# shubhamchandak94/Spring

Measured on AMD Instinct MI355X. Metric: Mreads/s through reorder stage, higher is better.
Workload: dtype u64; 1 GPU; 100000000 x 150 bp single-end synthetic reads per GPU (uniform genome 600000000 bp, 25x coverage, 1.0% substitutions, 50% reverse-complemented), inputs resident in HBM as .dna records; reads_per_gpu=100000000, read_len=150, chains=65536, num_thr=8, parallelism=single GPU, unmatched=13958636, singletons=12720853, rounds=1984, chain_groups=2

## Files before the change

### include/spring_reorder.h

```cpp
#ifndef SPRING_REORDER_H_
#define SPRING_REORDER_H_

#include <stddef.h>
#include <stdint.h>

#ifdef __cplusplus
extern "C" {
#endif

#define SPRING_REORDER_E_ARG (-1)
#define SPRING_REORDER_E_IO (-2)
#define SPRING_REORDER_E_HIP (-3)
#define SPRING_REORDER_E_STATE (-4)

typedef struct spring_reorder_ctx spring_reorder_ctx;

typedef struct {
  int32_t device;
  uint32_t num_chains;
  int32_t num_thr;
  int32_t collect_stats;
  int32_t time_search;
  int32_t force_literal_update;
  int32_t rounds_per_sync;
// ... 92 lines not shown
int spring_reorder_mg_slice(spring_reorder_ctx *ctx, void **d_prop, size_t *slice_off, size_t *slice_bytes,
                            size_t *total_bytes);
int spring_reorder_mg_slices(spring_reorder_ctx *ctx, void **d_prop, size_t slice_off[2], size_t slice_bytes[2],
                             size_t *total_bytes, uint32_t *count);
int spring_reorder_mg_apply(spring_reorder_ctx *ctx, int32_t check_alive, uint32_t *alive);
int spring_reorder_mg_end(spring_reorder_ctx *ctx);
int spring_reorder_debug_check_seed_state(spring_reorder_ctx *ctx, int32_t group, uint64_t *violations);
int spring_reorder_mg_exchange_virtual(spring_reorder_ctx **ctxs, uint32_t world);

#define SPRING_RCCL_ID_BYTES 128
typedef struct spring_mg_comm spring_mg_comm;
typedef int (*spring_mg_allgather_fn)(void *host_buf, size_t slice_off, size_t slice_bytes, size_t total_bytes,
                                      void *user);
int spring_mg_rccl_unique_id(void *id128);
int spring_mg_comm_create_rccl(spring_mg_comm **comm, int32_t device, const void *id128, uint32_t rank, uint32_t world);
int spring_mg_comm_create_host(spring_mg_comm **comm, spring_mg_allgather_fn fn, void *user, uint32_t rank,
                               uint32_t world);
void spring_mg_comm_destroy(spring_mg_comm *comm);
int spring_reorder_mg_run(spring_reorder_ctx *ctx, spring_mg_comm *comm, uint32_t total_chains);

int spring_reorder_finalize(spring_reorder_ctx *ctx);

int spring_reorder_get_stats(spring_reorder_ctx *ctx, spring_reorder_stats *st);

int spring_reorder_download(spring_reorder_ctx *ctx, uint32_t *order, char *rc, char *flag, int64_t *pos,
                            uint16_t *rlen, uint32_t *order_s, uint64_t *tid_off, uint64_t *tid_off_s);
int spring_reorder_tid_split(spring_reorder_ctx *ctx, uint64_t *mid, uint64_t *mid_s);

int spring_reorder_emit_dna(spring_reorder_ctx *ctx, int32_t tid, uint8_t *dst, size_t cap, size_t *nbytes);

int spring_reorder_dict_lookup(spring_reorder_ctx *ctx, int32_t which, const uint64_t *keys, uint32_t nkeys,
                               uint32_t *bin_size, uint32_t *bin_ids, size_t ids_cap);

int spring_reorder_download_reads(spring_reorder_ctx *ctx, uint64_t *limbs , uint16_t *len);

int spring_order_invert_se(const uint32_t *order, uint32_t n, uint32_t *order_array, double *kernel_ms);
int spring_order_invert_pe(const uint32_t *order, uint32_t n, uint32_t *order_array, double *kernel_ms);
int spring_order_correct(uint32_t *order, uint64_t m, const uint32_t *order_N, uint32_t nN, uint32_t n_clean,
                         double *kernel_ms);
int spring_order_pe_encode(const uint32_t *order, uint32_t n, uint32_t *new_order, double *kernel_ms);

int spring_fastq_reorder(const uint8_t *fastq, size_t nbytes, const uint32_t *order, uint32_t n, uint8_t *out,
                         size_t out_cap, size_t *out_bytes, double *kernel_ms);

#define SPRING_SYNTH_REPEATS 0x80000000u
#define SPRING_SYNTH_PAIRED 0x40000000u
#define SPRING_SYNTH_GENOMIC 0x20000000u
size_t spring_synth_dna_bytes(uint32_t n, uint32_t L);
int spring_synth_dna_host(uint8_t *dst, uint32_t n, uint32_t L, uint64_t G, uint64_t seed, uint32_t err_ppm);
int spring_synth_genome_host(uint8_t *dst, uint64_t G, uint64_t seed, uint32_t flags);
int spring_synth_dna_device(void *d_dst, uint32_t n, uint32_t L, uint64_t G, uint64_t seed, uint32_t err_ppm);
int spring_reorder_load_synth(spring_reorder_ctx *ctx, uint32_t n, uint32_t L, uint64_t G, uint64_t seed,
                              uint32_t err_ppm);
int spring_reorder_download_dna(spring_reorder_ctx *ctx, uint8_t *dst, size_t cap);

#ifdef __cplusplus
}
#endif
#endif
```

### spring_amd/_lib.py

```python
import ctypes as C
import os

HERE = os.path.dirname(os.path.abspath(__file__))
LIB_PATH = os.environ.get("SPRING_AMD_LIB") or os.path.join(HERE, "lib", "libspring_reorder_hip.so")

EXPORTS = [
    "spring_reorder_default_opts", "spring_reorder_last_error", "spring_reorder_trim_pool", "spring_reorder_run", "spring_reorder_create",
    "spring_reorder_destroy", "spring_reorder_load_dna", "spring_reorder_load_dna_device",
    "spring_reorder_build_dict", "spring_reorder_run_chains", "spring_reorder_auto_chains", "spring_reorder_finalize",
    "spring_reorder_mg_begin", "spring_reorder_mg_search", "spring_reorder_mg_slice", "spring_reorder_mg_slices",
    "spring_reorder_mg_apply",
    "spring_reorder_mg_end", "spring_reorder_mg_exchange_virtual", "spring_reorder_debug_check_seed_state",
    "spring_mg_rccl_unique_id", "spring_mg_comm_create_rccl", "spring_mg_comm_create_host", "spring_mg_comm_destroy",
    "spring_reorder_mg_run",
    "spring_reorder_get_stats", "spring_reorder_download", "spring_reorder_tid_split", "spring_reorder_emit_dna",
    "spring_reorder_dict_lookup", "spring_reorder_download_reads", "spring_synth_dna_bytes",
    "spring_reorder_load_fastq", "spring_reorder_fastq_N",
    "spring_order_invert_se", "spring_order_invert_pe", "spring_order_correct", "spring_order_pe_encode",
    "spring_fastq_reorder",
    "spring_synth_dna_host", "spring_synth_genome_host", "spring_synth_dna_device", "spring_reorder_load_synth", "spring_reorder_download_dna",
    "spring_encoder_create", "spring_encoder_destroy", "spring_encoder_set_split_tables", "spring_encoder_encode_reorder", "spring_encoder_download",
    "spring_encoder_download_seq_packed", "spring_encoder_get_info", "spring_reorder_encode_run", "spring_encoder_encode_host", "spring_encoder_run",
]

STREAMS_EXPORTS = [
    "spring_streams_create", "spring_streams_destroy", "spring_streams_from_encoder", "spring_streams_from_host",
    "spring_streams_download", "spring_streams_get_info", "spring_streams_run",
]
STREAMS_NUM = 9

DECODE_EXPORTS = [
    "spring_decode_create", "spring_decode_destroy", "spring_decode_seq_from_encoder", "spring_decode_seq_from_host",
    "spring_decode_seq_from_files", "spring_decode_from_streams", "spring_decode_from_host", "spring_decode_from_files",
    "spring_decode_download", "spring_decode_get_info",
]

QUALID_EXPORTS = [
    "spring_qualid_create", "spring_qualid_destroy", "spring_qualid_order_from_host", "spring_qualid_order_from_encoder",
    "spring_qualid_from_fastq", "spring_qualid_from_lines", "spring_qualid_download", "spring_qualid_get_info",
    "spring_quality_table", "spring_id_pattern",
]

FASTQ_OUT_EXPORTS = [
    "spring_fastq_out_create", "spring_fastq_out_destroy", "spring_fastq_out_assemble", "spring_fastq_out_download",
    "spring_fastq_out_write", "spring_fastq_out_get_info",
]

GZIP_EXPORTS = [
    "spring_gzip_create", "spring_gzip_destroy", "spring_gzip_set_chunk_bytes", "spring_gzip_from_fastq_out",
# ... 189 lines not shown
    L.spring_reorder_last_error.restype = C.c_char_p
    L.spring_reorder_trim_pool.restype = None
    L.spring_reorder_run.argtypes = [C.c_char_p, C.c_uint32, C.c_int32, C.c_int32, C.c_uint32, C.c_uint32,
                                     C.POINTER(Opts)]
    L.spring_reorder_create.argtypes = [C.POINTER(vp), C.POINTER(Opts)]
    L.spring_reorder_destroy.argtypes = [vp]
    L.spring_reorder_destroy.restype = None
    L.spring_reorder_load_dna.argtypes = [vp, u8p, C.c_size_t, C.c_uint32, C.c_uint32]
    L.spring_reorder_load_dna_device.argtypes = [vp, vp, C.c_size_t, C.c_uint32, C.c_uint32, C.c_int32]
    L.spring_reorder_build_dict.argtypes = [vp]
    L.spring_reorder_run_chains.argtypes = [vp]
    L.spring_reorder_auto_chains.argtypes = [vp, C.POINTER(C.c_uint32), C.POINTER(C.c_int32)]
    L.spring_reorder_finalize.argtypes = [vp]
    L.spring_reorder_mg_begin.argtypes = [vp, C.c_uint32, C.c_uint32, C.c_uint32, vp]
    L.spring_reorder_mg_search.argtypes = [vp]
    L.spring_reorder_mg_slice.argtypes = [vp, C.POINTER(vp), C.POINTER(C.c_size_t), C.POINTER(C.c_size_t), C.POINTER(C.c_size_t)]
    L.spring_reorder_mg_slices.argtypes = [vp, C.POINTER(vp), C.POINTER(C.c_size_t), C.POINTER(C.c_size_t), C.POINTER(C.c_size_t),
                                           C.POINTER(C.c_uint32)]
    L.spring_reorder_debug_check_seed_state.argtypes = [vp, C.c_int32, C.POINTER(C.c_uint64)]
    L.spring_reorder_mg_apply.argtypes = [vp, C.c_int32, C.POINTER(C.c_uint32)]
    L.spring_reorder_mg_end.argtypes = [vp]
    L.spring_reorder_mg_exchange_virtual.argtypes = [C.POINTER(vp), C.c_uint32]
    L.spring_mg_rccl_unique_id.argtypes = [vp]
    L.spring_mg_comm_create_rccl.argtypes = [C.POINTER(vp), C.c_int32, vp, C.c_uint32, C.c_uint32]
    L.spring_mg_comm_create_host.argtypes = [C.POINTER(vp), MG_ALLGATHER_FN, vp, C.c_uint32, C.c_uint32]
    L.spring_mg_comm_destroy.argtypes = [vp]
    L.spring_mg_comm_destroy.restype = None
    L.spring_reorder_mg_run.argtypes = [vp, vp, C.c_uint32]
    L.spring_reorder_get_stats.argtypes = [vp, C.POINTER(Stats)]
    L.spring_reorder_download.argtypes = [vp] + [vp] * 8
    L.spring_reorder_tid_split.argtypes = [vp, vp, vp]
    L.spring_reorder_emit_dna.argtypes = [vp, C.c_int32, u8p, C.c_size_t, C.POINTER(C.c_size_t)]
    L.spring_reorder_dict_lookup.argtypes = [vp, C.c_int32, vp, C.c_uint32, vp, vp, C.c_size_t]
    L.spring_reorder_download_reads.argtypes = [vp, vp, vp]
    L.spring_reorder_load_fastq.argtypes = [vp, vp, C.c_size_t, vp, C.c_size_t, C.POINTER(FastqInfo)]
    L.spring_reorder_fastq_N.argtypes = [vp, C.c_int32, vp, C.c_size_t, C.POINTER(C.c_size_t), vp, C.POINTER(C.c_uint32)]
    L.spring_order_invert_se.argtypes = [vp, C.c_uint32, vp, C.POINTER(C.c_double)]
    L.spring_order_invert_pe.argtypes = [vp, C.c_uint32, vp, C.POINTER(C.c_double)]
    L.spring_fastq_reorder.argtypes = [u8p, C.c_size_t, vp, C.c_uint32, u8p, C.c_size_t, C.POINTER(C.c_size_t),
                                       C.POINTER(C.c_double)]
    L.spring_order_pe_encode.argtypes = [vp, C.c_uint32, vp, C.POINTER(C.c_double)]
    L.spring_order_correct.argtypes = [vp, C.c_uint64, vp, C.c_uint32, C.c_uint32, C.POINTER(C.c_double)]
    L.spring_synth_dna_bytes.restype = C.c_size_t
    L.spring_synth_dna_bytes.argtypes = [C.c_uint32, C.c_uint32]
    L.spring_synth_dna_host.argtypes = [u8p, C.c_uint32, C.c_uint32, C.c_uint64, C.c_uint64, C.c_uint32]
    L.spring_synth_genome_host.argtypes = [u8p, C.c_uint64, C.c_uint64, C.c_uint32]
    L.spring_synth_dna_device.argtypes = [vp, C.c_uint32, C.c_uint32, C.c_uint64, C.c_uint64, C.c_uint32]
    L.spring_reorder_load_synth.argtypes = [vp, C.c_uint32, C.c_uint32, C.c_uint64, C.c_uint64, C.c_uint32]
    L.spring_reorder_download_dna.argtypes = [vp, u8p, C.c_size_t]
    L.spring_encoder_create.argtypes = [C.c_int32, C.POINTER(vp)]
    L.spring_encoder_destroy.argtypes = [vp]
    L.spring_encoder_destroy.restype = None
    L.spring_encoder_encode_reorder.argtypes = [vp, vp, u8p, C.c_uint64, vp, C.c_uint32, C.POINTER(EncoderInfo)]
    L.spring_encoder_download.argtypes = [vp] + [vp] * 9
    L.spring_encoder_download_seq_packed.argtypes = [vp, vp, vp]
    L.spring_encoder_encode_host.argtypes = [vp, C.c_uint32, C.c_int32, vp, u8p, C.c_uint64, vp, vp, vp, vp, vp, u8p,
                                             C.c_uint64, vp, C.c_uint32, u8p, C.c_uint64, vp, C.c_uint32,
                                             C.POINTER(EncoderInfo)]
    L.spring_encoder_run.argtypes = [C.c_char_p, C.c_uint32, C.c_int32, C.c_uint32, C.c_uint32, C.c_int32,
                                     C.POINTER(EncoderInfo)]
    L.spring_encoder_get_info.argtypes = [vp, C.POINTER(EncoderInfo)]
    L.spring_reorder_encode_run.argtypes = [C.c_char_p, C.c_uint32, C.c_int32, C.c_int32, C.c_uint32, C.c_uint32,
                                            C.c_uint32, C.POINTER(Opts), C.POINTER(EncoderInfo)]
    L.spring_streams_create.argtypes = [C.c_int32, C.POINTER(vp)]
    L.spring_streams_destroy.argtypes = [vp]
    L.spring_streams_destroy.restype = None
# ... 104 lines not shown
```

### spring_amd/csrc/dict_build.h

```cpp
#ifndef SPRING_DICT_BUILD_H_
#define SPRING_DICT_BUILD_H_

#include "reorder_device.h"

namespace sr {

bool launch_unpack_keys(hipStream_t st, const uint8_t *dna, uint32_t n, int L, int W, int S, uint32_t rec_fixed,
                        uint64_t *reads, uint16_t *lens, uint32_t *bad_len, int dstart0, int dend0, int dstart1, int dend1,
                        uint64_t *keys0, uint32_t *vals0, uint64_t *keys1, uint32_t *vals1);

constexpr int TAB_WRITE_LG = 10;
inline int tab_write_lg(int bshift) { return 64 - bshift < TAB_WRITE_LG ? 64 - bshift : TAB_WRITE_LG; }
inline uint32_t tab_write_blocks(int bshift) { return (uint32_t)(1ull << (64 - bshift - tab_write_lg(bshift))); }
void launch_tab_partition(hipStream_t st, const uint64_t *h0, uint32_t nk0, const uint64_t *h1, uint32_t nk1, int bshift,
                          uint32_t *part);
constexpr uint32_t TAB_OVF_SLOTS = 8;
void launch_tab_write(hipStream_t st, const uint64_t *h0, uint32_t nk0, const uint64_t *h1, uint32_t nk1,
                      const uint32_t *part, DictBuild d0, DictBuild d1, uint4 *fpt, int bshift, uint32_t *ovf,
                      uint32_t *ovf_blk, uint32_t *ovf_cnt);
void launch_tab_overflow_blocks(hipStream_t st, const uint64_t *h0, uint32_t nk0, const uint64_t *h1, DictBuild d0,
                                DictBuild d1, uint32_t *fpt, int bshift, const uint32_t *ovf_blk, const uint32_t *ovf_cnt);
void launch_tab_overflow_pairs(hipStream_t st, const uint64_t *h0, uint32_t nk0, const uint64_t *h1, DictBuild d0,
                               DictBuild d1, uint32_t *fpt, int bshift, const uint32_t *ovf, uint32_t novf);

constexpr uint32_t PRES_DROP_CTRS = 1024;
void launch_pres_insert(hipStream_t st, const uint64_t *h0, uint32_t nk0, const uint64_t *h1, uint32_t nk1, int wl, uint32_t *pres,
                        int lgb, uint32_t *drops);

}

#endif
```

### spring_amd/csrc/dict_build.hip

```cpp
#include <hip/hip_runtime.h>

#include "dict_build.h"
#include "strand_filter.h"

namespace sr {

__device__ __forceinline__ uint64_t db_mix64(uint64_t x) {
  x ^= x >> 33; x *= 0xff51afd7ed558ccdull; x ^= x >> 33; x *= 0xc4ceb9fe1a85ec53ull; x ^= x >> 33;
  return x;
}
__device__ __forceinline__ uint64_t db_unmix64(uint64_t x) {
  x ^= x >> 33; x *= 0x9cb4b2f8129337dbull; x ^= x >> 33; x *= 0x4f74430c22a54005ull; x ^= x >> 33;
  return x;
}
__device__ __forceinline__ uint32_t db_fp30_of(uint64_t h) {
  const uint32_t f = (uint32_t)h & 0x3fffffffu;
  return f == 0u ? 1u : f == 0x3fffffffu ? 0x3ffffffeu : f;
}

__global__ __launch_bounds__(256) void k_unpack_fixed_keys(const uint8_t *__restrict__ dna, uint32_t n, int L, int W, int lgS,
                                                           uint32_t rec, uint64_t *__restrict__ reads,
                                                           uint16_t *__restrict__ lens, uint32_t *__restrict__ bad_len,
                                                           int dstart0, int klen0, int dstart1, int klen1,
                                                           uint64_t *__restrict__ keys0, uint32_t *__restrict__ vals0,
// ... 233 lines not shown
  if (t >= ovf[0]) return;
  tab_overflow_insert(ovf[1u + t], h0, nk0, h1, d0, d1, fpt, bshift);
}

void launch_tab_partition(hipStream_t st, const uint64_t *h0, uint32_t nk0, const uint64_t *h1, uint32_t nk1, int bshift,
                          uint32_t *part) {
  const uint32_t nblk = tab_write_blocks(bshift);
  const uint64_t nt = 2ull * ((uint64_t)nblk + 1);
  hipLaunchKernelGGL(k_tab_partition, dim3((unsigned)((nt + 255) / 256)), dim3(256), 0, st, h0, nk0, h1, nk1, bshift,
                     tab_write_lg(bshift), nblk, part);
}
void launch_tab_write(hipStream_t st, const uint64_t *h0, uint32_t nk0, const uint64_t *h1, uint32_t nk1,
                      const uint32_t *part, DictBuild d0, DictBuild d1, uint4 *fpt, int bshift, uint32_t *ovf,
                      uint32_t *ovf_blk, uint32_t *ovf_cnt) {
  const uint32_t nblk = tab_write_blocks(bshift);
  hipLaunchKernelGGL(k_tab_write, dim3(nblk), dim3(TAB_WRITE_THREADS), 0, st, h0, nk0, h1, nk1, part, nblk, d0, d1, fpt, bshift,
                     tab_write_lg(bshift), ovf, ovf_blk, ovf_cnt);
}
void launch_tab_overflow_blocks(hipStream_t st, const uint64_t *h0, uint32_t nk0, const uint64_t *h1, DictBuild d0,
                                DictBuild d1, uint32_t *fpt, int bshift, const uint32_t *ovf_blk, const uint32_t *ovf_cnt) {
  const uint32_t nblk = tab_write_blocks(bshift);
  const uint64_t nt = (uint64_t)nblk * TAB_OVF_SLOTS;
  hipLaunchKernelGGL(k_tab_overflow_blocks, dim3((unsigned)((nt + 255) / 256)), dim3(256), 0, st, h0, nk0, h1, d0, d1, fpt, bshift,
                     nblk, ovf_blk, ovf_cnt);
}
void launch_tab_overflow_pairs(hipStream_t st, const uint64_t *h0, uint32_t nk0, const uint64_t *h1, DictBuild d0,
                               DictBuild d1, uint32_t *fpt, int bshift, const uint32_t *ovf, uint32_t novf) {
  if (!novf) return;
  hipLaunchKernelGGL(k_tab_overflow_pairs, dim3((novf + 255) / 256), dim3(256), 0, st, h0, nk0, h1, d0, d1, fpt, bshift, ovf);
}

__global__ __launch_bounds__(256) void k_pres_insert(const uint64_t *__restrict__ h0, uint32_t nk0, const uint64_t *__restrict__ h1,
                                                     uint32_t nk1, int wl, uint32_t *__restrict__ pres, int lgb,
                                                     uint32_t *__restrict__ drops) {
  __shared__ uint32_t s_drop;
  if (threadIdx.x == 0) s_drop = 0u;
  __syncthreads();
  const uint64_t t = (uint64_t)blockIdx.x * blockDim.x + threadIdx.x;
  if (t < (uint64_t)nk0 + nk1) {
    const int l = t >= nk0 ? 1 : 0;
    const uint64_t key = db_unmix64(l ? h1[t - nk0] : h0[t]);
    uint32_t flags;
    const uint64_t hc = sf::mix64(sf::canon_and_flags(key, wl, l, flags));
    const uint32_t fp = sf::fp_of(hc), word = (fp << 4) | flags;
    uint32_t *bk = pres + 4ull * sf::bucket_of(hc, lgb);
    bool placed = false;
    for (int sl = 0; sl < 4 && !placed; sl++) {
      uint32_t old = __hip_atomic_load(bk + sl, __ATOMIC_RELAXED, __HIP_MEMORY_SCOPE_AGENT);
      if (old == 0u) old = atomicCAS(bk + sl, 0u, word);
      if (old == 0u) placed = true;
      else if ((old >> 4) == fp) {
        if ((old & word & 15u) != (word & 15u)) atomicOr(bk + sl, word & 15u);
        placed = true;
      }
    }
    if (!placed) atomicAdd(&s_drop, 1u);
  }
  __syncthreads();
  if (threadIdx.x == 0 && s_drop) atomicAdd(drops + (blockIdx.x & (PRES_DROP_CTRS - 1u)), s_drop);
}
void launch_pres_insert(hipStream_t st, const uint64_t *h0, uint32_t nk0, const uint64_t *h1, uint32_t nk1, int wl, uint32_t *pres,
                        int lgb, uint32_t *drops) {
  const uint64_t nt = (uint64_t)nk0 + nk1;
  if (!nt) return;
  hipLaunchKernelGGL(k_pres_insert, dim3((unsigned)((nt + 255) / 256)), dim3(256), 0, st, h0, nk0, h1, nk1, wl, pres, lgb, drops);
}

}
```

### spring_amd/csrc/reorder_pipeline.cpp

```cpp
#include <hip/hip_runtime.h>
#include <dlfcn.h>

#include <algorithm>
#include <system_error>
#include <thread>
#include <memory>
#include <atomic>
#include <chrono>
#include <cstdarg>
#include <cstdio>
#include <cstdlib>
#include <cstring>
#include <map>
#include <mutex>
#include <new>
#include <stdexcept>
#include <string>
#include <unordered_map>
#include <vector>
#include <zlib.h>

#include "reorder_device.h"
#include "dict_build.h"
#include "reorder_internal.h"
// ... 965 lines not shown
  HIPCHK(hipStreamSynchronize(ctx->st));
  if (!ctx->n) return 0;
  if (limbs)
    HIPCHK(hipMemcpy2D(limbs, (size_t)ctx->W * 8, ctx->d_reads, (size_t)ctx->S * 8, (size_t)ctx->W * 8, ctx->n,
                       hipMemcpyDeviceToHost));
  if (len) HIPCHK(hipMemcpy(len, ctx->d_lens, (size_t)ctx->n * 2, hipMemcpyDeviceToHost));
  return 0;
}

static uint64_t pow2ceil(uint64_t x) {
  uint64_t p = 1;
  while (p < x) p <<= 1;
  return p;
}

static double now_ms() {
  return std::chrono::duration<double, std::milli>(std::chrono::steady_clock::now().time_since_epoch()).count();
}
#define DBG_T(label)                                                                         \
  do {                                                                                       \
    if (dbg) { (void)hipStreamSynchronize(st); double t_ = now_ms(); fprintf(stderr, "[dict] %-14s %8.2f ms\n", label, t_ - t_last); t_last = t_; } \
  } while (0)

static TabView tab_view(const spring_reorder_ctx *ctx) {
  TabView t;
  t.buck = ctx->fpt;
  t.bshift = ctx->bshift; t.minz = ctx->minz; t.lshift = ctx->lshift;
  return t;
}

static unsigned sort_prefix_auto(uint64_t m) { return m <= (1ull << 29) ? 40u : 48u; }

static bool strand_filter_wanted(const spring_reorder_ctx *ctx);
int spring_reorder_build_dict(spring_reorder_ctx *ctx) {
  double t_last = now_ms();
  if (!ctx) return fail(SPRING_REORDER_E_ARG, "ctx is NULL");
  const bool dbg = ctx->o.debug != 0;
  if (ctx->stage != ST_LOADED) return fail(SPRING_REORDER_E_STATE, "build_dict: load reads first");
  HIPCHK(hipSetDevice(ctx->dev));
  hipStream_t st = ctx->st;
  const uint32_t n = ctx->n;
  HIPCHK(hipEventRecord(ctx->ev[2], st));
  uint64_t *uhash[2] = {nullptr, nullptr};
  uint32_t *ustart[2] = {nullptr, nullptr}, *ucount[2] = {nullptr, nullptr};
  const bool both_dense = n && ctx->uniform && ctx->L > ctx->dict[0].end && ctx->L > ctx->dict[1].end;
  uint64_t *keys_both[2] = {nullptr, nullptr};
  uint32_t *vals_both[2] = {nullptr, nullptr};
  ctx->stats.dict_build_path = 0;
  if (both_dense && ctx->pre_keys[0] && ctx->o.dict_build_mode != 1) {
    for (int l = 0; l < 2; l++) {
      keys_both[l] = ctx->pre_keys[l]; vals_both[l] = ctx->pre_vals[l];
      ctx->pre_keys[l] = nullptr; ctx->pre_vals[l] = nullptr;
    }
    ctx->stats.dict_build_path |= 1;
  } else {
    drop_pre_keys(ctx);
  }
  ctx->stats.sort_repaired_runs = 0; ctx->stats.sort_full_sorts = 0; ctx->stats.sort_prefix_bits = 0;
  ctx->stats.sort_long_runs = 0; ctx->stats.sort_list_overflows = 0;
  for (int l = 0; l < 2; l++) {
    DictDev &d = ctx->dict[l];
    uint32_t m = 0;
    uint32_t *d_slot = nullptr, *d_flag = nullptr;
    void *d_tmp = nullptr;
    size_t tmp_bytes = 0;
    if (n) {
// ... 94 lines not shown
    HIPCHK(rle(st, d_tmp, tmp_bytes, k_out, m, k_in, cnt, d_nruns));
    uint32_t numkeys = 0;
    HIPCHK(hipMemcpyAsync(&numkeys, d_nruns, 4, hipMemcpyDeviceToHost, st));
    HIPCHK(hipStreamSynchronize(st));
    ctx->dfree(d_tmp); d_tmp = nullptr;
    ctx->dfree(k_out); ctx->dfree(d_nruns);
    d.numkeys = numkeys;
    DBG_T("rle");
    DMALLOC(ustart[l], (size_t)numkeys * 4);
    tmp_bytes = 0;
    HIPCHK(excl_scan_u32(st, nullptr, tmp_bytes, cnt, ustart[l], numkeys));
    DMALLOC(d_tmp, tmp_bytes);
    HIPCHK(excl_scan_u32(st, d_tmp, tmp_bytes, cnt, ustart[l], numkeys));
    DBG_T("scan");
    uhash[l] = k_in;
    ucount[l] = cnt;
    DMALLOC(d.urec, (size_t)numkeys * 16);
    DMALLOC(d.deep, ((size_t)m / DEEP_BIN + 1) * 4);
    DMALLOC(d.d_ndeep, 16);
    HIPCHK(hipMemsetAsync(d.d_ndeep, 0, 12, st));
    HIPCHK(hipStreamSynchronize(st));
    ctx->dfree(d_tmp);
    if (d_flag) { ctx->dfree(d_flag); ctx->dfree(d_slot); }
  }
  const uint64_t nk0 = ctx->dict[0].numkeys, nk1 = ctx->dict[1].numkeys, nm = nk0 + nk1;
  const int tab_scale = ctx->o.tab_scale > 0 ? ctx->o.tab_scale : 2;
  const uint64_t nb = std::max<uint64_t>(8, pow2ceil(std::max<uint64_t>(2, (nm * 10 + 15) / 16)) * (uint64_t)pow2ceil(tab_scale));
  ctx->bshift = 64;
  for (uint64_t v = nb; v > 1; v >>= 1) ctx->bshift--;
  ctx->minz = (ctx->dict[0].end - ctx->dict[0].start + 1 == MINZ_WL && ctx->L <= 192 && ctx->o.table_mode == 2) ? 1 : 0;
  ctx->lshift = 32 - (64 - ctx->bshift - 2);
  if (ctx->lshift < 1) return fail(SPRING_REORDER_E_ARG, "build_dict: table too large for minimizer addressing");
  ctx->stats.table_minz = ctx->minz; ctx->stats.table_marked_lines = 0;
  DMALLOC(ctx->fpt, nb * 32);
  const bool one_pass = nm && !ctx->minz && ctx->o.dict_build_mode != 1;
  if (!one_pass) HIPCHK(hipMemsetAsync(ctx->fpt, 0, nb * 32, st));
  uint32_t *const tab_words = reinterpret_cast<uint32_t *>(ctx->fpt);
  DBG_T("alloc+memset tab");
  if (one_pass) {
    if (nm >= 0xffffffffull) return fail(SPRING_REORDER_E_ARG, "build_dict: %llu keys exceed the 32-bit index space of the table build", (unsigned long long)nm);
    ctx->stats.dict_build_path |= 2;
    ctx->marked_lines = 0;
    DictBuild db[2];
    for (int l = 0; l < 2; l++) {
      DictDev &d = ctx->dict[l];
      db[l].ustart = ustart[l]; db[l].ucount = ucount[l]; db[l].ids = d.ids; db[l].urec = d.urec;
      db[l].deep = d.deep; db[l].ndeep = d.d_ndeep;
    }
    uint32_t *d_part = nullptr, *d_ovf = nullptr, *d_ovf_blk = nullptr, *d_ovf_cnt = nullptr, novf = 0;
    const size_t nblk = tab_write_blocks(ctx->bshift);
    DMALLOC(d_part, 2 * (nblk + 1) * 4);
    DMALLOC(d_ovf_blk, nblk * TAB_OVF_SLOTS * 4);
    DMALLOC(d_ovf_cnt, nblk * 4);
    DMALLOC(d_ovf, ((size_t)nm + 1) * 4);
    HIPCHK(hipMemsetAsync(d_ovf, 0, 4, st));
    launch_tab_partition(st, uhash[0], (uint32_t)nk0, uhash[1], (uint32_t)nk1, ctx->bshift, d_part);
    launch_tab_write(st, uhash[0], (uint32_t)nk0, uhash[1], (uint32_t)nk1, d_part, db[0], db[1], ctx->fpt, ctx->bshift, d_ovf,
                     d_ovf_blk, d_ovf_cnt);
    launch_tab_overflow_blocks(st, uhash[0], (uint32_t)nk0, uhash[1], db[0], db[1], tab_words, ctx->bshift, d_ovf_blk, d_ovf_cnt);
    HIPCHK(hipGetLastError());
    HIPCHK(hipMemcpyAsync(&novf, d_ovf, 4, hipMemcpyDeviceToHost, st));
    uint32_t nd[2][3] = {{0, 0, 0}, {0, 0, 0}};
    for (int l = 0; l < 2; l++)
      HIPCHK(hipMemcpyAsync(nd[l], ctx->dict[l].d_ndeep, 12, hipMemcpyDeviceToHost, st));
    HIPCHK(hipStreamSynchronize(st));
    DBG_T("table write");
// ... 50 lines not shown
      DBG_T("insert pass 0");
      launch_tab_overflow(st, h_in, v_in, nm, db[0], db[1], tab_words, ctx->bshift, d_ovf, novf);
      if (dbg) fprintf(stderr, "[dict] %u of %llu pairs overflow their bucket\n", novf, (unsigned long long)nm);
    } else {
      DMALLOC(bk_in, nm * 4); DMALLOC(bk_out, nm * 4);
      DMALLOC(tp_in, nm * 8); DMALLOC(tp_out, nm * 8);
      launch_minz_prepare(st, h_in, v_in, nm, db[0], db[1], ctx->lshift, bk_in, tp_in);
      DBG_T("minz prepare");
      const unsigned end_bit = (unsigned)(64 - ctx->bshift);
      size_t tb = 0;
      HIPCHK(sort_pairs_u32_u64(st, nullptr, tb, bk_in, bk_out, tp_in, tp_out, nm, end_bit));
      DMALLOC(d_tmp2, tb);
      HIPCHK(sort_pairs_u32_u64(st, d_tmp2, tb, bk_in, bk_out, tp_in, tp_out, nm, end_bit));
      DBG_T("minz sort");
      DMALLOC(d_marked, 16);
      HIPCHK(hipMemsetAsync(d_marked, 0, 4, st));
      launch_tab_insert_minz(st, bk_out, tp_out, nm, tab_words, ctx->bshift, d_marked);
      HIPCHK(hipMemcpyAsync(&ctx->marked_lines, d_marked, 4, hipMemcpyDeviceToHost, st));
    }
    HIPCHK(hipGetLastError());
    uint32_t nd[2][3] = {{0, 0, 0}, {0, 0, 0}};
    for (int l = 0; l < 2; l++)
      HIPCHK(hipMemcpyAsync(nd[l], ctx->dict[l].d_ndeep, 12, hipMemcpyDeviceToHost, st));
    HIPCHK(hipStreamSynchronize(st));
    for (int l = 0; l < 2; l++) { ctx->dict[l].ndeep = nd[l][0]; ctx->dict[l].big_reads = nd[l][1]; ctx->dict[l].mid_reads = nd[l][2]; }
    if (dbg) fprintf(stderr, "[dict] reads %u + %u, keys %u + %u, bins >= %u: %u + %u, reads in bins >= %u: %u + %u, >= %u: %u + %u\n",
                     ctx->dict[0].numreads, ctx->dict[1].numreads, ctx->dict[0].numkeys, ctx->dict[1].numkeys, DEEP_BIN, nd[0][0], nd[1][0],
                     MID_BIN, nd[0][2], nd[1][2], BIG_BIN, nd[0][1], nd[1][1]);
    ctx->stats.table_marked_lines = ctx->marked_lines;
    DBG_T("insert");
    ctx->dfree(mv0); ctx->dfree(mh); ctx->dfree(mv); ctx->dfree(d_tmp);
    ctx->dfree(bk_in); ctx->dfree(bk_out); ctx->dfree(tp_in); ctx->dfree(tp_out); ctx->dfree(d_tmp2); ctx->dfree(d_marked); ctx->dfree(d_ovf);
  }
  ctx->pres = nullptr; ctx->pres_lgb = 0;
  ctx->stats.strand_filter = 0; ctx->stats.strand_filter_dropped = 0;
  int lgb = 0;
  if (nm && nm < 0xffffffffull && strand_filter_wanted(ctx)) {
    while (lgb < 32 && (1ull << lgb) < nm) lgb++;
    if (ctx->o.strand_filter > 0) lgb = std::min(lgb, ctx->o.strand_filter);
    if (ctx->dmalloc((void **)&ctx->pres, (size_t)16 << lgb)) {
      (void)hipGetLastError();
      ctx->pres = nullptr;
      if (dbg) fprintf(stderr, "[dict] presence table: no room for 2^%d buckets, running without\n", lgb);
    }
  }
  if (ctx->pres) {
    uint32_t *d_drops = nullptr;
    std::vector<uint32_t> h_drops(PRES_DROP_CTRS);
    DMALLOC(d_drops, PRES_DROP_CTRS * 4);
    HIPCHK(hipMemsetAsync(ctx->pres, 0, (size_t)16 << lgb, st));
    HIPCHK(hipMemsetAsync(d_drops, 0, PRES_DROP_CTRS * 4, st));
    launch_pres_insert(st, uhash[0], (uint32_t)nk0, uhash[1], (uint32_t)nk1, ctx->dict[0].end - ctx->dict[0].start + 1,
                       reinterpret_cast<uint32_t *>(ctx->pres), lgb, d_drops);
    HIPCHK(hipGetLastError());
    HIPCHK(hipMemcpyAsync(h_drops.data(), d_drops, PRES_DROP_CTRS * 4, hipMemcpyDeviceToHost, st));
    HIPCHK(hipStreamSynchronize(st));
    for (uint32_t v : h_drops) ctx->stats.strand_filter_dropped += v;
    ctx->pres_lgb = lgb;
    ctx->dfree(d_drops);
    if (dbg) fprintf(stderr, "[dict] presence table: 2^%d buckets, %llu of %llu keys dropped\n", lgb,
                     (unsigned long long)ctx->stats.strand_filter_dropped, (unsigned long long)nm);
    DBG_T("presence table");
  }
  for (int l = 0; l < 2; l++) { ctx->dfree(uhash[l]); ctx->dfree(ustart[l]); ctx->dfree(ucount[l]); }
  DBG_T("free temps");
  HIPCHK(hipEventRecord(ctx->ev[3], st));
  ctx->stage = ST_DICT;
  return 0;
}

int spring_reorder_dict_lookup(spring_reorder_ctx *ctx, int32_t which, const uint64_t *keys, uint32_t nkeys,
                               uint32_t *bin_size, uint32_t *bin_ids, size_t ids_cap) {
  if (!ctx || ctx->stage < ST_DICT) return fail(SPRING_REORDER_E_STATE, "dict_lookup: build_dict first");
  if (which < 0 || which > 1) return fail(SPRING_REORDER_E_ARG, "which must be 0 or 1");
  HIPCHK(hipSetDevice(ctx->dev));
  DictDev &d = ctx->dict[which];
  uint64_t *dk = nullptr;
  uint32_t *ds = nullptr, *dc = nullptr;
  DMALLOC(dk, (size_t)nkeys * 8);
  DMALLOC(ds, (size_t)nkeys * 4);
  DMALLOC(dc, (size_t)nkeys * 4);
  std::vector<uint32_t> hs(nkeys), hc(nkeys), hids(d.numreads);
  if (nkeys) {
    HIPCHK(hipMemcpyAsync(dk, keys, (size_t)nkeys * 8, hipMemcpyHostToDevice, ctx->st));
    launch_dict_lookup(ctx->st, tab_view(ctx), d.urec, which, ctx->d_reads, ctx->S, d.start, d.end, dk, nkeys, ds, dc);
    HIPCHK(hipMemcpyAsync(hs.data(), ds, (size_t)nkeys * 4, hipMemcpyDeviceToHost, ctx->st));
    HIPCHK(hipMemcpyAsync(hc.data(), dc, (size_t)nkeys * 4, hipMemcpyDeviceToHost, ctx->st));
  }
  if (d.numreads) HIPCHK(hipMemcpyAsync(hids.data(), d.ids, (size_t)d.numreads * 4, hipMemcpyDeviceToHost, ctx->st));
  HIPCHK(hipStreamSynchronize(ctx->st));
  ctx->dfree(dk); ctx->dfree(ds); ctx->dfree(dc);
  size_t o = 0;
  for (uint32_t i = 0; i < nkeys; i++) {
    if (hc[i] != 0xffffffffu && (hc[i] & 0x80000000u)) {
      bin_size[i] = 1;
      if (o + 1 > ids_cap) return fail(SPRING_REORDER_E_ARG, "bin_ids too small");
      bin_ids[o++] = hs[i];
      continue;
    }
    bin_size[i] = hc[i];
// ... 1352 lines not shown
```

### spring_amd/csrc/strand_filter.h

```cpp
#ifndef SPRING_STRAND_FILTER_H_
#define SPRING_STRAND_FILTER_H_

#include <stdint.h>

#if defined(__HIPCC__) || defined(__CUDACC__)
#define SF_FN __host__ __device__ inline
#else
#define SF_FN inline
#endif

namespace sf {

SF_FN uint64_t mix64(uint64_t x) {
  x ^= x >> 33; x *= 0xff51afd7ed558ccdull; x ^= x >> 33; x *= 0xc4ceb9fe1a85ec53ull; x ^= x >> 33;
  return x;
}
SF_FN uint64_t brev64(uint64_t x) {
  x = ((x >> 1) & 0x5555555555555555ull) | ((x & 0x5555555555555555ull) << 1);
  x = ((x >> 2) & 0x3333333333333333ull) | ((x & 0x3333333333333333ull) << 2);
  x = ((x >> 4) & 0x0f0f0f0f0f0f0f0full) | ((x & 0x0f0f0f0f0f0f0f0full) << 4);
  x = ((x >> 8) & 0x00ff00ff00ff00ffull) | ((x & 0x00ff00ff00ff00ffull) << 8);
  x = ((x >> 16) & 0x0000ffff0000ffffull) | ((x & 0x0000ffff0000ffffull) << 16);
  return (x >> 32) | (x << 32);
}
SF_FN uint64_t rc_window(uint64_t w, int wl) {
#if defined(__HIP_DEVICE_COMPILE__)
  uint64_t x = __builtin_bitreverse64(w);
#else
  uint64_t x = brev64(w);
#endif
  x = ((x >> 1) & 0x5555555555555555ull) | ((x & 0x5555555555555555ull) << 1);
  return ~x >> (64 - 2 * wl);
}
SF_FN int rc_limb_bitpos(int R, int j) { return 2 * (R - 32 - 32 * j); }
SF_FN uint64_t rc_limb(uint64_t w, int nv) {
  return rc_window(w, 32) & (nv >= 32 ? ~0ull : ((1ull << (2 * nv)) - 1));
}
SF_FN uint64_t canon(uint64_t w, int wl, bool &swapped) {
  const uint64_t r = rc_window(w, wl);
  swapped = r < w;
  return swapped ? r : w;
}
SF_FN uint32_t bucket_of(uint64_t h, int lgb) { return lgb ? (uint32_t)(h >> (64 - lgb)) : 0u; }
SF_FN uint32_t fp_of(uint64_t h) {
  const uint32_t f = (uint32_t)h & 0x0fffffffu;
  return f ? f : 1u;
}
SF_FN uint64_t canon_and_flags(uint64_t w, int wl, int l, uint32_t &flags) {
  const uint64_t r = rc_window(w, wl);
  flags = (w <= r ? 1u << l : 0u) | (r <= w ? 4u << l : 0u);
  return r < w ? r : w;
}
SF_FN uint32_t flags_of_key(uint64_t w, int wl, int l) {
  uint32_t f;
  (void)canon_and_flags(w, wl, l, f);
  return f;
}
SF_FN uint32_t absent_of(uint32_t s0, uint32_t s1, uint32_t s2, uint32_t s3, uint32_t fp) {
  const uint32_t f0 = (s0 >> 4) == fp ? s0 : 0u, f1 = (s1 >> 4) == fp ? s1 : 0u, f2 = (s2 >> 4) == fp ? s2 : 0u,
                 f3 = (s3 >> 4) == fp ? s3 : 0u;
  const uint32_t hit = f0 | f1 | f2 | f3;
  return s3 != 0u ? 0u : ~hit & 15u;
}
SF_FN uint32_t to_window_frame(uint32_t a, bool swapped) { return swapped ? ((a >> 2) | (a << 2)) & 15u : a; }

}

#endif
```

### spring_amd/reorder.py

```python
import ctypes as C
from dataclasses import dataclass

import numpy as np

from . import _lib


class ReorderError(RuntimeError):
    """Raised where the reference throws std::runtime_error (call_template_functions.cpp:60)."""


@dataclass
class ReorderOpts:
    device: int = -1
    num_chains: int = 0
    num_thr: int = 1
    collect_stats: bool = False
    time_search: bool = False
    force_literal_update: bool = False
    rounds_per_sync: int = 0
    first_shifts: int = 0
    seed_wide: int = 0
    tab_scale: int = 0
    search_wpb: int = 0
# ... 150 lines not shown

    def streams(self):
        st = self.stats()
        nm, ns, T = st["n_matched"], st["n_single"], self.opts.num_thr
        out = dict(order=np.zeros(max(nm, 1), np.uint32), rc=np.zeros(max(nm, 1), np.uint8),
                   flag=np.zeros(max(nm, 1), np.uint8), pos=np.zeros(max(nm, 1), np.int64),
                   rlen=np.zeros(max(nm, 1), np.uint16), order_s=np.zeros(max(ns, 1), np.uint32),
                   tid_off=np.zeros(T + 1, np.uint64), tid_off_s=np.zeros(T + 1, np.uint64))
        _chk(self._L.spring_reorder_download(self._h, *[out[k].ctypes.data for k in (
            "order", "rc", "flag", "pos", "rlen", "order_s", "tid_off", "tid_off_s")]))
        for k in ("order", "rc", "flag", "pos", "rlen"):
            out[k] = out[k][:nm]
        out["order_s"] = out["order_s"][:ns]
        out["tid_mid"], out["tid_mid_s"] = np.zeros(T, np.uint64), np.zeros(T, np.uint64)
        _chk(self._L.spring_reorder_tid_split(self._h, out["tid_mid"].ctypes.data, out["tid_mid_s"].ctypes.data))
        out["stats"] = st
        return out

    def emit_dna(self, tid: int) -> bytes:
        nb = C.c_size_t()
        _chk(self._L.spring_reorder_emit_dna(self._h, tid, None, 0, C.byref(nb)))
        buf = np.zeros(max(nb.value, 1), np.uint8)
        _chk(self._L.spring_reorder_emit_dna(self._h, tid, buf.ctypes.data, nb.value, C.byref(nb)))
        return buf[:nb.value].tobytes()

    def dict_lookup(self, which, keys):
        keys = np.ascontiguousarray(keys, dtype=np.uint64)
        sizes = np.zeros(max(len(keys), 1), np.uint32)
        ids = np.zeros(max(self.n, 1) * 2, np.uint32)
        _chk(self._L.spring_reorder_dict_lookup(self._h, which, keys.ctypes.data, len(keys), sizes.ctypes.data,
                                                ids.ctypes.data, len(ids)))
        return sizes[:len(keys)], ids

    def download_reads(self):
        W = (2 * self.max_readlen - 1) // 64 + 1
        limbs = np.zeros((max(self.n, 1), W), np.uint64)
        ln = np.zeros(max(self.n, 1), np.uint16)
        _chk(self._L.spring_reorder_download_reads(self._h, limbs.ctypes.data, ln.ctypes.data))
        return limbs[:self.n], ln[:self.n]

    def download_dna(self) -> bytes:
        nb = self._L.spring_synth_dna_bytes(self.n, self.max_readlen)
        buf = np.zeros(max(nb, 1), np.uint8)
        _chk(self._L.spring_reorder_download_dna(self._h, buf.ctypes.data, nb))
        p = 0
        for _ in range(self.n):
            p += 2 + ((int(buf[p]) | (int(buf[p + 1]) << 8)) + 3) // 4
        return buf[:p].tobytes()


def reorder_dna(dna: bytes, n: int, max_readlen: int, opts: ReorderOpts = None):
    with ReorderStage(opts) as s:
        s.load_dna(dna, n, max_readlen)
        return s.run().streams()


def synth_dna_host(n, L, G, seed, err_ppm=10000) -> bytes:
    L_ = _lib.lib()
    nb = L_.spring_synth_dna_bytes(n, L)
    buf = np.zeros(max(nb, 1), np.uint8)
    _chk(L_.spring_synth_dna_host(buf.ctypes.data, n, L, G, seed, err_ppm))
    return buf[:nb].tobytes()


SYNTH_REPEATS = 0x80000000
SYNTH_PAIRED = 0x40000000
# ... 27 lines not shown
```

Baseline: 358.1 Mreads/s.

## Build strand presence table by streaming per-block LDS images instead of global atomics

Builds the strand-filter presence table by partitioning sorted key hashes into bucket ranges, inserting each range into an LDS image and writing the image out contiguously. This removes the global memset and the scattered global atomics for most keys. Keys whose canonical form is swapped are inserted afterwards by the old atomic kernel. It adds a partition kernel, a second pass over the keys, and a dump API used for validation.

```diff
diff --git a/include/spring_reorder.h b/include/spring_reorder.h
--- a/include/spring_reorder.h
+++ b/include/spring_reorder.h
@@ -148,6 +148,8 @@
 int spring_reorder_dict_lookup(spring_reorder_ctx *ctx, int32_t which, const uint64_t *keys, uint32_t nkeys,
                                uint32_t *bin_size, uint32_t *bin_ids, size_t ids_cap);
 
+int spring_reorder_pres_dump(spring_reorder_ctx *ctx, uint32_t *out, size_t cap_bytes, int32_t *lgb);
+
 int spring_reorder_download_reads(spring_reorder_ctx *ctx, uint64_t *limbs , uint16_t *len);
 
 int spring_order_invert_se(const uint32_t *order, uint32_t n, uint32_t *order_array, double *kernel_ms);
diff --git a/spring_amd/_lib.py b/spring_amd/_lib.py
--- a/spring_amd/_lib.py
+++ b/spring_amd/_lib.py
@@ -14,7 +14,7 @@
     "spring_mg_rccl_unique_id", "spring_mg_comm_create_rccl", "spring_mg_comm_create_host", "spring_mg_comm_destroy",
     "spring_reorder_mg_run",
     "spring_reorder_get_stats", "spring_reorder_download", "spring_reorder_tid_split", "spring_reorder_emit_dna",
-    "spring_reorder_dict_lookup", "spring_reorder_download_reads", "spring_synth_dna_bytes",
+    "spring_reorder_dict_lookup", "spring_reorder_pres_dump", "spring_reorder_download_reads", "spring_synth_dna_bytes",
     "spring_reorder_load_fastq", "spring_reorder_fastq_N",
     "spring_order_invert_se", "spring_order_invert_pe", "spring_order_correct", "spring_order_pe_encode",
     "spring_fastq_reorder",
@@ -270,6 +270,7 @@
     L.spring_reorder_tid_split.argtypes = [vp, vp, vp]
     L.spring_reorder_emit_dna.argtypes = [vp, C.c_int32, u8p, C.c_size_t, C.POINTER(C.c_size_t)]
     L.spring_reorder_dict_lookup.argtypes = [vp, C.c_int32, vp, C.c_uint32, vp, vp, C.c_size_t]
+    L.spring_reorder_pres_dump.argtypes = [vp, vp, C.c_size_t, C.POINTER(C.c_int32)]
     L.spring_reorder_download_reads.argtypes = [vp, vp, vp]
     L.spring_reorder_load_fastq.argtypes = [vp, vp, C.c_size_t, vp, C.c_size_t, C.POINTER(FastqInfo)]
     L.spring_reorder_fastq_N.argtypes = [vp, C.c_int32, vp, C.c_size_t, C.POINTER(C.c_size_t), vp, C.POINTER(C.c_uint32)]
diff --git a/spring_amd/csrc/dict_build.h b/spring_amd/csrc/dict_build.h
--- a/spring_amd/csrc/dict_build.h
+++ b/spring_amd/csrc/dict_build.h
@@ -2,6 +2,7 @@
 #define SPRING_DICT_BUILD_H_
 
 #include "reorder_device.h"
+#include "strand_filter.h"
 
 namespace sr {
 
@@ -25,7 +26,13 @@
 
 constexpr uint32_t PRES_DROP_CTRS = 1024;
 void launch_pres_insert(hipStream_t st, const uint64_t *h0, uint32_t nk0, const uint64_t *h1, uint32_t nk1, int wl, uint32_t *pres,
-                        int lgb, uint32_t *drops);
+                        int lgb, uint32_t *drops, bool swapped_only = false, uint32_t *n_swapped = nullptr);
+
+constexpr int PRES_WRITE_LG = sf::WRITE_LG;
+inline bool pres_write_applies(int lgb, uint64_t nkeys) { return sf::write_applies(lgb, nkeys); }
+inline uint32_t pres_write_blocks(int lgb) { return 1u << (lgb - PRES_WRITE_LG); }
+void launch_pres_write(hipStream_t st, const uint64_t *h0, uint32_t nk0, const uint64_t *h1, uint32_t nk1, int wl, uint4 *pres,
+                       int lgb, uint32_t *part, uint32_t *drops);
 
 }
 
diff --git a/spring_amd/csrc/dict_build.hip b/spring_amd/csrc/dict_build.hip
--- a/spring_amd/csrc/dict_build.hip
+++ b/spring_amd/csrc/dict_build.hip
@@ -289,38 +289,79 @@
 
 __global__ __launch_bounds__(256) void k_pres_insert(const uint64_t *__restrict__ h0, uint32_t nk0, const uint64_t *__restrict__ h1,
                                                      uint32_t nk1, int wl, uint32_t *__restrict__ pres, int lgb,
-                                                     uint32_t *__restrict__ drops) {
-  __shared__ uint32_t s_drop;
-  if (threadIdx.x == 0) s_drop = 0u;
+                                                     uint32_t *__restrict__ drops, bool swapped_only,
+                                                     uint32_t *__restrict__ n_swapped) {
+  __shared__ uint32_t s_drop, s_swapped;
+  if (threadIdx.x == 0) { s_drop = 0u; s_swapped = 0u; }
   __syncthreads();
   const uint64_t t = (uint64_t)blockIdx.x * blockDim.x + threadIdx.x;
   if (t < (uint64_t)nk0 + nk1) {
     const int l = t >= nk0 ? 1 : 0;
     const uint64_t key = db_unmix64(l ? h1[t - nk0] : h0[t]);
     uint32_t flags;
-    const uint64_t hc = sf::mix64(sf::canon_and_flags(key, wl, l, flags));
-    const uint32_t fp = sf::fp_of(hc), word = (fp << 4) | flags;
-    uint32_t *bk = pres + 4ull * sf::bucket_of(hc, lgb);
-    bool placed = false;
-    for (int sl = 0; sl < 4 && !placed; sl++) {
-      uint32_t old = __hip_atomic_load(bk + sl, __ATOMIC_RELAXED, __HIP_MEMORY_SCOPE_AGENT);
-      if (old == 0u) old = atomicCAS(bk + sl, 0u, word);
-      if (old == 0u) placed = true;
-      else if ((old >> 4) == fp) {
-        if ((old & word & 15u) != (word & 15u)) atomicOr(bk + sl, word & 15u);
-        placed = true;
-      }
-    }
-    if (!placed) atomicAdd(&s_drop, 1u);
+    const uint64_t c = sf::canon_and_flags(key, wl, l, flags);
+    const bool swapped = !((flags >> l) & 1u);
+    if (n_swapped && swapped) atomicAdd(&s_swapped, 1u);
+    if (!swapped_only || swapped) {
+      const uint64_t hc = sf::mix64(c);
+      if (!sf::place(pres + 4ull * sf::bucket_of(hc, lgb), (sf::fp_of(hc) << 4) | flags)) atomicAdd(&s_drop, 1u);
+    }
   }
   __syncthreads();
   if (threadIdx.x == 0 && s_drop) atomicAdd(drops + (blockIdx.x & (PRES_DROP_CTRS - 1u)), s_drop);
+  if (threadIdx.x == 0 && s_swapped) atomicAdd(n_swapped + (blockIdx.x & (PRES_DROP_CTRS - 1u)), s_swapped);
 }
 void launch_pres_insert(hipStream_t st, const uint64_t *h0, uint32_t nk0, const uint64_t *h1, uint32_t nk1, int wl, uint32_t *pres,
-                        int lgb, uint32_t *drops) {
+                        int lgb, uint32_t *drops, bool swapped_only, uint32_t *n_swapped) {
   const uint64_t nt = (uint64_t)nk0 + nk1;
   if (!nt) return;
-  hipLaunchKernelGGL(k_pres_insert, dim3((unsigned)((nt + 255) / 256)), dim3(256), 0, st, h0, nk0, h1, nk1, wl, pres, lgb, drops);
-}
-
-}
+  hipLaunchKernelGGL(k_pres_insert, dim3((unsigned)((nt + 255) / 256)), dim3(256), 0, st, h0, nk0, h1, nk1, wl, pres, lgb, drops,
+                     swapped_only, n_swapped);
+}
+
+constexpr uint32_t PRES_WRITE_THREADS = 256;
+__global__ __launch_bounds__(PRES_WRITE_THREADS) void k_pres_write(const uint64_t *__restrict__ h0, const uint64_t *__restrict__ h1,
+                                                                   const uint32_t *__restrict__ part, uint32_t nblk, int wl,
+                                                                   uint4 *__restrict__ pres, int lgb, uint32_t *__restrict__ drops) {
+  constexpr uint32_t NBK = 1u << PRES_WRITE_LG;
+  __shared__ uint4 img[NBK];
+  __shared__ uint32_t s_drop;
+  const uint32_t blk = blockIdx.x;
+  for (uint32_t k = threadIdx.x; k < NBK; k += PRES_WRITE_THREADS) img[k] = make_uint4(0u, 0u, 0u, 0u);
+  if (threadIdx.x == 0) s_drop = 0u;
+  const uint32_t a0 = part[blk], a1 = part[(uint64_t)nblk + 1 + blk];
+  const uint32_t c0 = part[blk + 1] - a0, c1 = part[(uint64_t)nblk + 2 + blk] - a1;
+  const uint32_t ntot = c0 + c1;
+  __syncthreads();
+  uint32_t *imgw = reinterpret_cast<uint32_t *>(img);
+  auto hash_of = [&](uint32_t t) -> uint64_t { return t >= c0 ? h1[a1 + (t - c0)] : h0[a0 + t]; };
+  auto enter = [&](uint32_t t, uint64_t h) {
+    const int l = t >= c0 ? 1 : 0;
+    uint32_t flags;
+    const uint64_t key = db_unmix64(h);
+    (void)sf::canon_and_flags(key, wl, l, flags);
+    if (!((flags >> l) & 1u)) return;
+    const uint32_t bl = sf::bucket_of(h, lgb) & (NBK - 1u);
+    if (!sf::place(imgw + 4u * bl, (sf::fp_of(h) << 4) | flags)) atomicAdd(&s_drop, 1u);
+  };
+  for (uint64_t t = threadIdx.x; t < ntot; t += 2u * PRES_WRITE_THREADS) {
+    const uint64_t t1 = t + PRES_WRITE_THREADS;
+    const uint64_t ha = hash_of((uint32_t)t), hb = t1 < ntot ? hash_of((uint32_t)t1) : 0ull;
+    enter((uint32_t)t, ha);
+    if (t1 < ntot) enter((uint32_t)t1, hb);
+  }
+  __syncthreads();
+  uint4 *__restrict__ out = pres + ((uint64_t)blk << PRES_WRITE_LG);
+  for (uint32_t k = threadIdx.x; k < NBK; k += PRES_WRITE_THREADS) out[k] = img[k];
+  if (threadIdx.x == 0 && s_drop) atomicAdd(drops + (blk & (PRES_DROP_CTRS - 1u)), s_drop);
+}
+void launch_pres_write(hipStream_t st, const uint64_t *h0, uint32_t nk0, const uint64_t *h1, uint32_t nk1, int wl, uint4 *pres,
+                       int lgb, uint32_t *part, uint32_t *drops) {
+  const uint32_t nblk = pres_write_blocks(lgb);
+  const uint64_t nt = 2ull * ((uint64_t)nblk + 1);
+  hipLaunchKernelGGL(k_tab_partition, dim3((unsigned)((nt + 255) / 256)), dim3(256), 0, st, h0, nk0, h1, nk1, 64 - lgb, PRES_WRITE_LG,
+                     nblk, part);
+  hipLaunchKernelGGL(k_pres_write, dim3(nblk), dim3(PRES_WRITE_THREADS), 0, st, h0, h1, part, nblk, wl, pres, lgb, drops);
+}
+
+}
diff --git a/spring_amd/csrc/reorder_pipeline.cpp b/spring_amd/csrc/reorder_pipeline.cpp
--- a/spring_amd/csrc/reorder_pipeline.cpp
+++ b/spring_amd/csrc/reorder_pipeline.cpp
@@ -1021,6 +1021,64 @@
 static unsigned sort_prefix_auto(uint64_t m) { return m <= (1ull << 29) ? 40u : 48u; }
 
 static bool strand_filter_wanted(const spring_reorder_ctx *ctx);
+
+static int build_pres(spring_reorder_ctx *ctx, uint64_t *const uhash[2], uint64_t nk0, uint64_t nk1) {
+  const bool dbg = ctx->o.debug != 0;
+  const uint64_t nm = nk0 + nk1;
+  hipStream_t st = ctx->st;
+  if (!(nm && nm < 0xffffffffull && strand_filter_wanted(ctx))) return 0;
+  int lgb = 0;
+  while (lgb < 32 && (1ull << lgb) < nm) lgb++;
+  if (ctx->o.strand_filter > 0) lgb = std::min(lgb, ctx->o.strand_filter);
+  if (ctx->dmalloc((void **)&ctx->pres, (size_t)16 << lgb)) {
+    (void)hipGetLastError();
+    ctx->pres = nullptr;
+    if (dbg) fprintf(stderr, "[dict] presence table: no room for 2^%d buckets, running without\n", lgb);
+    return 0;
+  }
+  bool streamed = ctx->o.dict_build_mode != 1 && pres_write_applies(lgb, nm);
+  const int wl = ctx->dict[0].end - ctx->dict[0].start + 1;
+  uint32_t *d_ctrs = nullptr, *d_part = nullptr;
+  std::vector<uint32_t> h(2 * PRES_DROP_CTRS);
+  if (streamed && ctx->dmalloc((void **)&d_part, 2 * ((size_t)pres_write_blocks(lgb) + 1) * 4)) {
+    (void)hipGetLastError();
+    d_part = nullptr;
+    streamed = false;
+  }
+  if (ctx->dmalloc((void **)&d_ctrs, h.size() * 4)) {
+    (void)hipGetLastError();
+    ctx->dfree(d_part); ctx->dfree(ctx->pres);
+    ctx->pres = nullptr;
+    if (dbg) fprintf(stderr, "[dict] presence table: no room for its counters, running without\n");
+    return 0;
+  }
+  HIPCHK(hipMemsetAsync(d_ctrs, 0, h.size() * 4, st));
+  uint32_t *const words = reinterpret_cast<uint32_t *>(ctx->pres);
+  if (streamed) {
+    launch_pres_write(st, uhash[0], (uint32_t)nk0, uhash[1], (uint32_t)nk1, wl, ctx->pres, lgb, d_part, d_ctrs);
+    launch_pres_insert(st, uhash[0], (uint32_t)nk0, uhash[1], (uint32_t)nk1, wl, words, lgb, d_ctrs, true,
+                       dbg ? d_ctrs + PRES_DROP_CTRS : nullptr);
+  } else {
+    HIPCHK(hipMemsetAsync(ctx->pres, 0, (size_t)16 << lgb, st));
+    launch_pres_insert(st, uhash[0], (uint32_t)nk0, uhash[1], (uint32_t)nk1, wl, words, lgb, d_ctrs);
+  }
+  HIPCHK(hipGetLastError());
+  HIPCHK(hipMemcpyAsync(h.data(), d_ctrs, h.size() * 4, hipMemcpyDeviceToHost, st));
+  HIPCHK(hipStreamSynchronize(st));
+  for (uint32_t i = 0; i < PRES_DROP_CTRS; i++) ctx->stats.strand_filter_dropped += h[i];
+  ctx->pres_lgb = lgb;
+  ctx->dfree(d_ctrs); ctx->dfree(d_part);
+  if (dbg) {
+    fprintf(stderr, "[dict] presence table: 2^%d buckets, %llu of %llu keys dropped\n", lgb,
+            (unsigned long long)ctx->stats.strand_filter_dropped, (unsigned long long)nm);
+    uint64_t nsw = 0;
+    for (uint32_t i = 0; i < PRES_DROP_CTRS; i++) nsw += h[PRES_DROP_CTRS + i];
+    if (streamed) fprintf(stderr, "[dict] presence table: written as a stream, %llu of %llu keys (%.4f) inserted behind it\n",
+                          (unsigned long long)nsw, (unsigned long long)nm, (double)nsw / (double)nm);
+  }
+  return 0;
+}
+
 int spring_reorder_build_dict(spring_reorder_ctx *ctx) {
   double t_last = now_ms();
   if (!ctx) return fail(SPRING_REORDER_E_ARG, "ctx is NULL");
@@ -1181,6 +1239,8 @@
   ctx->lshift = 32 - (64 - ctx->bshift - 2);
   if (ctx->lshift < 1) return fail(SPRING_REORDER_E_ARG, "build_dict: table too large for minimizer addressing");
   ctx->stats.table_minz = ctx->minz; ctx->stats.table_marked_lines = 0;
+  ctx->pres = nullptr; ctx->pres_lgb = 0;
+  ctx->stats.strand_filter = 0; ctx->stats.strand_filter_dropped = 0;
   DMALLOC(ctx->fpt, nb * 32);
   const bool one_pass = nm && !ctx->minz && ctx->o.dict_build_mode != 1;
   if (!one_pass) HIPCHK(hipMemsetAsync(ctx->fpt, 0, nb * 32, st));
@@ -1297,40 +1357,29 @@
     ctx->dfree(mv0); ctx->dfree(mh); ctx->dfree(mv); ctx->dfree(d_tmp);
     ctx->dfree(bk_in); ctx->dfree(bk_out); ctx->dfree(tp_in); ctx->dfree(tp_out); ctx->dfree(d_tmp2); ctx->dfree(d_marked); ctx->dfree(d_ovf);
   }
-  ctx->pres = nullptr; ctx->pres_lgb = 0;
-  ctx->stats.strand_filter = 0; ctx->stats.strand_filter_dropped = 0;
-  int lgb = 0;
-  if (nm && nm < 0xffffffffull && strand_filter_wanted(ctx)) {
-    while (lgb < 32 && (1ull << lgb) < nm) lgb++;
-    if (ctx->o.strand_filter > 0) lgb = std::min(lgb, ctx->o.strand_filter);
-    if (ctx->dmalloc((void **)&ctx->pres, (size_t)16 << lgb)) {
-      (void)hipGetLastError();
-      ctx->pres = nullptr;
-      if (dbg) fprintf(stderr, "[dict] presence table: no room for 2^%d buckets, running without\n", lgb);
-    }
-  }
-  if (ctx->pres) {
-    uint32_t *d_drops = nullptr;
-    std::vector<uint32_t> h_drops(PRES_DROP_CTRS);
-    DMALLOC(d_drops, PRES_DROP_CTRS * 4);
-    HIPCHK(hipMemsetAsync(ctx->pres, 0, (size_t)16 << lgb, st));
-    HIPCHK(hipMemsetAsync(d_drops, 0, PRES_DROP_CTRS * 4, st));
-    launch_pres_insert(st, uhash[0], (uint32_t)nk0, uhash[1], (uint32_t)nk1, ctx->dict[0].end - ctx->dict[0].start + 1,
-                       reinterpret_cast<uint32_t *>(ctx->pres), lgb, d_drops);
-    HIPCHK(hipGetLastError());
-    HIPCHK(hipMemcpyAsync(h_drops.data(), d_drops, PRES_DROP_CTRS * 4, hipMemcpyDeviceToHost, st));
-    HIPCHK(hipStreamSynchronize(st));
-    for (uint32_t v : h_drops) ctx->stats.strand_filter_dropped += v;
-    ctx->pres_lgb = lgb;
-    ctx->dfree(d_drops);
-    if (dbg) fprintf(stderr, "[dict] presence table: 2^%d buckets, %llu of %llu keys dropped\n", lgb,
-                     (unsigned long long)ctx->stats.strand_filter_dropped, (unsigned long long)nm);
-    DBG_T("presence table");
-  }
+  {
+    int r = build_pres(ctx, uhash, nk0, nk1);
+    if (r) return r;
+  }
+  if (ctx->pres) DBG_T("presence table");
   for (int l = 0; l < 2; l++) { ctx->dfree(uhash[l]); ctx->dfree(ustart[l]); ctx->dfree(ucount[l]); }
   DBG_T("free temps");
   HIPCHK(hipEventRecord(ctx->ev[3], st));
   ctx->stage = ST_DICT;
+  return 0;
+}
+
+int spring_reorder_pres_dump(spring_reorder_ctx *ctx, uint32_t *out, size_t cap_bytes, int32_t *lgb) {
+  if (!ctx || !lgb) return fail(SPRING_REORDER_E_ARG, "NULL argument");
+  if (ctx->stage < ST_DICT) return fail(SPRING_REORDER_E_STATE, "pres_dump: build_dict first");
+  if (!ctx->pres) { *lgb = -1; return 0; }
+  *lgb = ctx->pres_lgb;
+  const size_t bytes = (size_t)16 << ctx->pres_lgb;
+  if (!out) return 0;
+  if (cap_bytes < bytes) return fail(SPRING_REORDER_E_ARG, "pres_dump: %zu bytes of room for a table of %zu", cap_bytes, bytes);
+  HIPCHK(hipSetDevice(ctx->dev));
+  HIPCHK(hipStreamSynchronize(ctx->st));
+  HIPCHK(hipMemcpy(out, ctx->pres, bytes, hipMemcpyDeviceToHost));
   return 0;
 }
 
diff --git a/spring_amd/csrc/strand_filter.h b/spring_amd/csrc/strand_filter.h
--- a/spring_amd/csrc/strand_filter.h
+++ b/spring_amd/csrc/strand_filter.h
@@ -56,6 +56,37 @@
   (void)canon_and_flags(w, wl, l, f);
   return f;
 }
+SF_FN bool place(uint32_t *bk, uint32_t word) {
+  const uint32_t fp = word >> 4, flags = word & 15u;
+  for (int sl = 0; sl < 4; sl++) {
+#if defined(__HIP_DEVICE_COMPILE__)
+    uint32_t old = __hip_atomic_load(bk + sl, __ATOMIC_RELAXED, __HIP_MEMORY_SCOPE_AGENT);
+    if (old == 0u) old = atomicCAS(bk + sl, 0u, word);
+#else
+    const uint32_t old = bk[sl];
+    if (old == 0u) bk[sl] = word;
+#endif
+    if (old == 0u) return true;
+    if ((old >> 4) == fp) {
+      if ((old & flags) != flags) {
+#if defined(__HIP_DEVICE_COMPILE__)
+        atomicOr(bk + sl, flags);
+#else
+        bk[sl] = old | flags;
+#endif
+      }
+      return true;
+    }
+  }
+  return false;
+}
+constexpr int WRITE_LG = 11;
+constexpr uint32_t WRITE_MIN_BLOCKS = 1024, WRITE_MAX_KEYS_PER_BLOCK = 2u << WRITE_LG;
+SF_FN bool write_applies(int lgb, uint64_t nkeys) {
+  if (lgb < WRITE_LG || lgb > 32) return false;
+  const uint64_t nblk = 1ull << (lgb - WRITE_LG);
+  return nblk >= WRITE_MIN_BLOCKS || nkeys <= nblk * WRITE_MAX_KEYS_PER_BLOCK;
+}
 SF_FN uint32_t absent_of(uint32_t s0, uint32_t s1, uint32_t s2, uint32_t s3, uint32_t fp) {
   const uint32_t f0 = (s0 >> 4) == fp ? s0 : 0u, f1 = (s1 >> 4) == fp ? s1 : 0u, f2 = (s2 >> 4) == fp ? s2 : 0u,
                  f3 = (s3 >> 4) == fp ? s3 : 0u;
diff --git a/spring_amd/reorder.py b/spring_amd/reorder.py
--- a/spring_amd/reorder.py
+++ b/spring_amd/reorder.py
@@ -206,6 +206,15 @@
                                                 ids.ctypes.data, len(ids)))
         return sizes[:len(keys)], ids
 
+    def pres_dump(self):
+        lgb = C.c_int32()
+        _chk(self._L.spring_reorder_pres_dump(self._h, None, 0, C.byref(lgb)))
+        if lgb.value < 0:
+            return None, -1
+        tab = np.zeros((1 << lgb.value, 4), np.uint32)
+        _chk(self._L.spring_reorder_pres_dump(self._h, tab.ctypes.data, tab.nbytes, C.byref(lgb)))
+        return tab, lgb.value
+
     def download_reads(self):
         W = (2 * self.max_readlen - 1) // 64 + 1
         limbs = np.zeros((max(self.n, 1), W), np.uint64)
```

After: 362.1 Mreads/s, median of 6. About the same (+1.1%).
